# dyollb/segmantic

Measured on AMD Instinct MI355X. Metric: 3D UNet train voxels/s on 128^3 bf16, higher is better.
Workload: dtype bf16

## Files before the change

segmantic_amd/csrc/conv_ring3_impl.h:

```cpp
#pragma once
#include "conv_ring_impl.h"

namespace segmi {

struct Ring3Geom {
  static constexpr int TD = 4, TH = 8, TW = 16, HH = TH + 2, HW = TW + 2;
  static constexpr int ROWB = 32;
  static constexpr int PLANE_ROWS = HH * HW;
  static constexpr int PLANE_B = PLANE_ROWS * ROWB;
  static constexpr int PLANE_CH = PLANE_ROWS * 2;
  static constexpr int GROUP_CH = TD * PLANE_CH;
  static constexpr int GROUP_B = GROUP_CH * 16 + 512;
  static constexpr int NG = 3;
  static constexpr int RING_B = NG * GROUP_B;
  static constexpr int NPIECE = (GROUP_CH + 63) / 64;
  static constexpr int NDMA = (NPIECE + 3) / 4;
  static constexpr int TFS_OFF = RING_B, BPRM_OFF = TFS_OFF + 128, DUMP_OFF = BPRM_OFF + 256;
  static constexpr int LDS_BYTES = DUMP_OFF + 256 * 16;
};

__device__ __forceinline__ void ring3_dma16(const __amdgpu_buffer_rsrc_t rs, unsigned lds_addr, unsigned voff,
                                            unsigned soff) {
  unsigned keep;
  asm volatile(
      "s_mov_b32 %0, m0\n\ts_mov_b32 m0, %1\n\ts_nop 0\n\tbuffer_load_dwordx4 %2, %3, %4 offen lds\n\ts_mov_b32 m0, %0"
      : "=&s"(keep)
      : "s"(lds_addr), "v"(voff), "s"(rs), "s"(soff)
      : "memory");
}

template <typename T, int MODE>
__global__ __launch_bounds__(256, 2) void conv_ring3_kernel(ConvParams p) {
  using G = Ring3Geom;
  constexpr int J = 5;
  constexpr int NIT = 6 * J;
  constexpr unsigned kOob = 0x80000000u;
  extern __shared__ __attribute__((aligned(16))) char smem[];
  const int tid = threadIdx.x, lane = tid & 63;
  const int wave = __builtin_amdgcn_readfirstlane(tid >> 6);
  const int g = lane >> 4, r = lane & 15;

  int t = blockIdx.x;
  if (p.xcd) t = (t & 7) * (gridDim.x >> 3) + (t >> 3);
  const int seg = t % p.tz; t /= p.tz;
  const int txi = t % p.tx; t /= p.tx;
  const int tyi = t % p.ty;
  const int n = t / p.ty;
  const int oy0 = tyi * G::TH, ox0 = txi * G::TW;
  const int nt0 = blockIdx.y;
  const int total_steps = (p.Do + G::TD - 1) / G::TD;
  const int seg_steps = (total_steps + p.tz - 1) / p.tz;
  const int z0 = seg * seg_steps * G::TD;
  const int nsteps_z = total_steps - seg * seg_steps < seg_steps ? total_steps - seg * seg_steps : seg_steps;

  constexpr bool PLAIN = MODE == 0;
  constexpr bool BSUM = MODE == 4;
  constexpr bool has_alpha = (MODE & 1) != 0;
  constexpr bool want_stats = (MODE & 2) != 0;
  const T* resp = (const T*)p.res;
  const bool res_in = resp && p.res == p.in && p.ldr == p.ldi && p.Cin == p.Cout;
  const bool res_ext = resp && !res_in;

  frag_t wreg[3][J];
#pragma unroll
  for (int kd = 0; kd < 3; ++kd)
#pragma unroll
    for (int j = 0; j < J; ++j) {
      wreg[kd][j] = frag_t{0u, 0u, 0u, 0u};
      const int t9 = 2 * j + (g >> 1);
      if (t9 <= 8) {
        const int tap = kd * 9 + t9;
        const int sp = tap >> 1, gp = (tap & 1) * 2 + (g & 1);
        wreg[kd][j] = *reinterpret_cast<const frag_t*>(
            (const char*)p.wfrag + (((int64_t)sp * p.ntiles_total + nt0) * 64 + gp * 16 + r) * 16);
      }
    }
  int lb[J];
#pragma unroll
  for (int j = 0; j < J; ++j) {
    int t9 = 2 * j + (g >> 1);
    if (t9 > 8) t9 = 8;
    lb[j] = ((t9 / 3) * G::HW + t9 % 3 + r) * G::ROWB + (g & 1) * 16 + wave * 2 * G::HW * G::ROWB;
  }

  const int64_t plane_stride = (int64_t)p.Hi * p.Wi * p.ldi * (int64_t)sizeof(T);
  const unsigned plane_b32 = (unsigned)plane_stride;
  const char* img = (const char*)p.in + (int64_t)n * p.Di * plane_stride;
  const __amdgpu_buffer_rsrc_t rs_in =
      __builtin_amdgcn_make_buffer_rsrc((void*)img, 0, (int)((unsigned)p.Di * plane_b32), 0x00020000);
  unsigned goff[G::NDMA];
  unsigned gpl = 0;
  bool xy_inside = true;
#pragma unroll
  for (int mi = 0; mi < G::NDMA; ++mi) {
    const int i = 64 * (wave + 4 * mi) + lane;
    const int pl = i / G::PLANE_CH, rem = i % G::PLANE_CH;
    const int row = rem >> 1, ch = rem & 1;
    const int y = oy0 - 1 + row / G::HW, x = ox0 - 1 + row % G::HW;
    const bool ok = i < G::GROUP_CH && (unsigned)y < (unsigned)p.Hi && (unsigned)x < (unsigned)p.Wi;
    goff[mi] = ok ? (unsigned)pl * plane_b32 + (unsigned)((y * p.Wi + x) * p.ldi * (int)sizeof(T) + ch * 16) : kOob;
    gpl |= (unsigned)((pl & 3) | (ok ? 0 : 8)) << (4 * mi);
    xy_inside = xy_inside && (ok || i >= G::GROUP_CH);
  }
  const bool wave_inside = __builtin_amdgcn_readfirstlane(__all(xy_inside) ? 1 : 0) != 0;
  const unsigned lds0 = (unsigned)(uintptr_t)smem;
  const unsigned lds_wave = (unsigned)(1024 * wave);
  const bool last_piece = wave + 4 * (G::NDMA - 1) < G::NPIECE;
  auto dma_group = [&](unsigned gbase, int zfirst) {
    const unsigned soff = (unsigned)zfirst * plane_b32;
#pragma unroll
    for (int mi = 0; mi < G::NDMA; ++mi)
      if (mi < G::NDMA - 1 || last_piece) ring3_dma16(rs_in, lds0 + gbase + lds_wave + 4096u * mi, goff[mi], soff);
  };

  const bool in_tf = p.in_scale != nullptr;
  const bool in_act = in_tf && p.in_alpha != nullptr;
  float* tfs = reinterpret_cast<float*>(smem + G::TFS_OFF);
  if (in_tf && tid < 32) tfs[tid] = tid < 16 ? p.in_scale[tid] : p.in_shift[tid - 16];
  float in_alpha = in_act ? *p.in_alpha : 0.f;
  touch_s(in_alpha);
  const bool in_act01 = in_act && in_alpha >= 0.f && in_alpha <= 1.f;
  auto transform_group = [&](unsigned gbase, int zrem) {
    const int tfo = (lane & 1) * 32;
    float sc[8], sh[8];
    const char* tb = reinterpret_cast<const char*>(tfs);
#pragma unroll
    for (int e = 0; e < 8; e += 4) {
      *reinterpret_cast<f32x4*>(&sc[e]) = *reinterpret_cast<const f32x4*>(tb + tfo + e * 4);
      *reinterpret_cast<f32x4*>(&sh[e]) = *reinterpret_cast<const f32x4*>(tb + 64 + tfo + e * 4);
    }
    const unsigned mine = gbase + lds_wave + 16u * lane;
    const bool fast = zrem >= G::TD && wave_inside;
    auto run = [&](auto tf, auto dst) {
      frag_t raw[G::NDMA - 1];
#pragma unroll
      for (int mi = 0; mi < G::NDMA - 1; ++mi) raw[mi] = *reinterpret_cast<const frag_t*>(smem + mine + 4096u * mi);
      frag_t rawl = frag_t{0u, 0u, 0u, 0u};
      if (last_piece) rawl = *reinterpret_cast<const frag_t*>(smem + mine + 4096u * (G::NDMA - 1));
#pragma unroll
      for (int mi = 0; mi < G::NDMA - 1; ++mi)
        *reinterpret_cast<frag_t*>(smem + dst(mi, mine + 4096u * mi)) = tf(raw[mi]);
      const unsigned al = last_piece ? dst(G::NDMA - 1, mine + 4096u * (G::NDMA - 1)) : (unsigned)(G::DUMP_OFF + tid * 16);
      *reinterpret_cast<frag_t*>(smem + al) = tf(rawl);
    };
    auto with_dst = [&](auto tf) {
      if (fast) run(tf, [&](int, unsigned a) { return a; });
      else run(tf, [&](int mi, unsigned a) {
        const unsigned nib = (gpl >> (4 * mi)) & 15u;
        const bool keep = nib < 8u && (int)nib < zrem;
        return keep ? a : (unsigned)(G::DUMP_OFF + tid * 16);
      });
    };
    if (in_act01) with_dst([&](frag_t v) { return bn_prelu01_h8<T>(v, sc, sh, in_alpha); });
    else with_dst([&](frag_t v) { return bn_prelu_h8<T>(v, sc, sh, in_alpha, in_act); });
  };

  {
    const unsigned dst0 = 2u * G::GROUP_B + 2u * G::PLANE_B;
#pragma unroll
    for (int mi = 0; mi < 3; ++mi) {
      const int i = 64 * (wave + 4 * mi) + lane;
      const int pl = i / G::PLANE_CH, rem = i % G::PLANE_CH;
      const int row = rem >> 1, ch = rem & 1;
      const int z = z0 - 1 + pl, y = oy0 - 1 + row / G::HW, x = ox0 - 1 + row % G::HW;
      const bool ok = (unsigned)z < (unsigned)p.Di && (unsigned)y < (unsigned)p.Hi && (unsigned)x < (unsigned)p.Wi;
      const unsigned vo = ok ? (unsigned)z * plane_b32 + (unsigned)((y * p.Wi + x) * p.ldi * (int)sizeof(T) + ch * 16) : kOob;
      if (i < 2 * G::PLANE_CH) ring3_dma16(rs_in, lds0 + dst0 + 1024u * (wave + 4 * mi), vo, 0u);
    }
    dma_group(0u, z0 + 1);
    if (in_tf) {
      asm volatile("s_waitcnt vmcnt(0)" ::: "memory");
      __syncthreads();
      const int tfo = (lane & 1) * 32;
      float sc[8], sh[8];
#pragma unroll
      for (int e = 0; e < 8; ++e) { sc[e] = tfs[tfo / 4 + e]; sh[e] = tfs[16 + tfo / 4 + e]; }
#pragma unroll
      for (int mi = 0; mi < 3; ++mi) {
        const int i = 64 * (wave + 4 * mi) + lane;
        const int pl = i / G::PLANE_CH, row = (i % G::PLANE_CH) >> 1;
        const int z = z0 - 1 + pl, y = oy0 - 1 + row / G::HW, x = ox0 - 1 + row % G::HW;
        const bool ok = i < 2 * G::PLANE_CH && (unsigned)z < (unsigned)p.Di && (unsigned)y < (unsigned)p.Hi &&
                        (unsigned)x < (unsigned)p.Wi;
        if (ok) {
          frag_t* q = reinterpret_cast<frag_t*>(smem + dst0 + 16u * i);
          *q = bn_prelu_h8<T>(*q, sc, sh, in_alpha, in_act);
        }
      }
      transform_group(0u, p.Di - (z0 + 1));
    }
    asm volatile("s_waitcnt vmcnt(0) lgkmcnt(0)" ::: "memory");
    __syncthreads();
  }

  f32x4 bias4 = f32x4{0.f, 0.f, 0.f, 0.f};
  if (p.bias) bias4 = *reinterpret_cast<const f32x4*>(p.bias + nt0 * 16 + 4 * g);
  touch_v(bias4);
  float alpha = has_alpha ? *p.alpha : 0.f;
  touch_s(alpha);
  const bool alpha01 = has_alpha && alpha >= 0.f && alpha <= 1.f;
  f32x4 ssum = f32x4{0.f, 0.f, 0.f, 0.f}, ssq = ssum;
  f32x4 bs0 = ssum, bs1 = ssum, bs2 = ssum;
  float* bprm = reinterpret_cast<float*>(smem + G::BPRM_OFF);
  float balpha = 1.f;
  if constexpr (BSUM) {
    if (tid < 64) {
      const int which = tid / 16, ch = nt0 * 16 + tid % 16;
      const float mean = p.bmean[ch], istd = p.binvstd[ch];
      const float sc = istd * (p.bgamma ? p.bgamma[ch] : 1.f);
      bprm[tid] = which == 0 ? mean : which == 1 ? istd : which == 2 ? sc : fmaf(-mean, sc, p.bbeta ? p.bbeta[ch] : 0.f);
    }
    balpha = p.balpha ? *p.balpha : 1.f;
    touch_s(balpha);
    __syncthreads();
  }
  const bool b_has_alpha = BSUM && p.balpha != nullptr;
  const T* bxp = (const T*)p.bx;
  T* outp = (T*)p.out;
  const int co = nt0 * 16 + 4 * g;
  unsigned o_off[2], r_off[2], b_off[2];
  bool row_ok[2];
#pragma unroll
  for (int ro = 0; ro < 2; ++ro) {
    const int oy = oy0 + 2 * wave + ro, ox = ox0 + r;
    row_ok[ro] = oy < p.Ho && ox < p.Wo;
    o_off[ro] = row_ok[ro] ? (unsigned)((oy * p.Wo + ox) * p.ldo + co) * (unsigned)sizeof(T) : kOob;
    r_off[ro] = row_ok[ro] ? (unsigned)((oy * p.Wo + ox) * p.ldr + co) * (unsigned)sizeof(T) : kOob;
    b_off[ro] = row_ok[ro] ? (unsigned)((oy * p.Wo + ox) * p.ldbx + co) * (unsigned)sizeof(T) : kOob;
  }
  const int64_t oplane = (int64_t)p.Ho * p.Wo * p.ldo, rplane = (int64_t)p.Ho * p.Wo * p.ldr;
  const int64_t bplane = (int64_t)p.Ho * p.Wo * p.ldbx;
  const unsigned oplane_b = (unsigned)(oplane * (int64_t)sizeof(T)), rplane_b = (unsigned)(rplane * (int64_t)sizeof(T)),
                 bplane_b = (unsigned)(bplane * (int64_t)sizeof(T));
  const __amdgpu_buffer_rsrc_t rs_out = __builtin_amdgcn_make_buffer_rsrc(
      (void*)(outp + (int64_t)n * p.Do * oplane), 0, (int)((unsigned)p.Do * oplane_b), 0x00020000);
  const __amdgpu_buffer_rsrc_t rs_res = __builtin_amdgcn_make_buffer_rsrc(
      (void*)(res_ext ? resp + (int64_t)n * p.Do * rplane : (const T*)p.out), 0, res_ext ? (int)((unsigned)p.Do * rplane_b) : 0,
      0x00020000);
  const __amdgpu_buffer_rsrc_t rs_bx = __builtin_amdgcn_make_buffer_rsrc(
      (void*)(BSUM ? bxp + (int64_t)n * p.Do * bplane : (const T*)p.out), 0, BSUM ? (int)((unsigned)p.Do * bplane_b) : 0,
      0x00020000);

  unsigned g_prev = 2u * G::GROUP_B, g_cur = 0u, g_next = (unsigned)G::GROUP_B;
  for (int step = 0; step < nsteps_z; ++step) {
    const int zb = step * G::TD;
    const bool more = step + 1 < nsteps_z;
    if (more) dma_group(g_next, z0 + zb + 5);
    typedef typename Raw4<T>::type raw4_t;
    raw4_t resv[4][2];
    if (res_ext) {
#pragma unroll
      for (int zi = 0; zi < 4; ++zi)
#pragma unroll
        for (int ro = 0; ro < 2; ++ro)
          resv[zi][ro] = __builtin_amdgcn_raw_buffer_load_b64(rs_res, r_off[ro], (unsigned)(z0 + zb + zi) * rplane_b, 0);
    }
    raw4_t bxv[BSUM ? 4 : 1][2];
    auto fetch_bx = [&](int zi) {
#pragma unroll
      for (int ro = 0; ro < 2; ++ro)
        bxv[BSUM ? zi : 0][ro] =
            __builtin_amdgcn_raw_buffer_load_b64(rs_bx, b_off[ro], (unsigned)(z0 + zb + zi) * bplane_b, 0);
    };
    if constexpr (BSUM) { fetch_bx(0); fetch_bx(1); fetch_bx(2); fetch_bx(3); }

    int bp[J], bc[J];
#pragma unroll
    for (int j = 0; j < J; ++j) { bp[j] = lb[j] + (int)g_prev; bc[j] = lb[j] + (int)g_cur; }
    f32x4 acc[4][2];
    constexpr int PD = MODE == 4 ? 3 : 4;
    frag_t a[PD + 1][2];
    auto issue = [&](int it, frag_t (&dst)[2]) {
      const int c = it / J, j = it % J;
      const char* base = smem + (c < 2 ? bp[j] + (c + 2) * G::PLANE_B : bc[j] + (c - 2) * G::PLANE_B);
      dst[0] = *reinterpret_cast<const frag_t*>(base);
      dst[1] = *reinterpret_cast<const frag_t*>(base + G::HW * G::ROWB);
    };
#pragma unroll
    for (int q = 0; q < PD; ++q) issue(q, a[q]);
#pragma unroll
    for (int it = 0; it < NIT; ++it) {
      if (it + PD < NIT) issue(it + PD, a[(it + PD) % (PD + 1)]);
      __builtin_amdgcn_sched_barrier(0);
      const int c = it / J, j = it % J;
#pragma unroll
      for (int kd = 0; kd < 3; ++kd) {
        const int zi = c - kd;
        if (zi >= 0 && zi < 4) {
          const bool first = kd == 0 && j == 0;
          const f32x4 zero = f32x4{0.f, 0.f, 0.f, 0.f};
          acc[zi][0] = mma16<T>(wreg[kd][j], a[it % (PD + 1)][0], first ? zero : acc[zi][0]);
          acc[zi][1] = mma16<T>(wreg[kd][j], a[it % (PD + 1)][1], first ? zero : acc[zi][1]);
        }
      }
      __builtin_amdgcn_sched_barrier(0);
    }
    if (in_tf && more) {
      asm volatile("s_waitcnt vmcnt(0)" ::: "memory");
      transform_group(g_next, p.Di - (z0 + zb + 5));
    }
    if (res_in) {
#pragma unroll
      for (int zi = 0; zi < 4; ++zi)
#pragma unroll
        for (int ro = 0; ro < 2; ++ro) {
          const int c = zi + 1;
          const unsigned pb = c < 2 ? g_prev + (c + 2) * G::PLANE_B : g_cur + (c - 2) * G::PLANE_B;
          resv[zi][ro] = *reinterpret_cast<const raw4_t*>(
              smem + pb + ((2 * wave + ro + 1) * G::HW + r + 1) * G::ROWB + (4 * g) * (int)sizeof(T));
        }
    }
    if (resp) {
#pragma unroll
      for (int zi = 0; zi < 4; ++zi)
#pragma unroll
        for (int ro = 0; ro < 2; ++ro) touch_v(resv[zi][ro]);
    }
    f32x4 bsc4, bsh4, bmean4;
    if constexpr (BSUM) {
#pragma unroll
      for (int zi = 0; zi < 4; ++zi)
#pragma unroll
        for (int ro = 0; ro < 2; ++ro) touch_v(bxv[zi][ro]);
      bsc4 = *reinterpret_cast<const f32x4*>(bprm + 2 * 16 + 4 * g);
      bsh4 = *reinterpret_cast<const f32x4*>(bprm + 3 * 16 + 4 * g);
      bmean4 = *reinterpret_cast<const f32x4*>(bprm + 4 * g);
    }
#pragma unroll
    for (int zi = 0; zi < 4; ++zi) {
      const int oz = z0 + zb + zi;
      const unsigned opoff = (unsigned)oz * oplane_b;
      const bool zin_out = oz < p.Do;
#pragma unroll
      for (int ro = 0; ro < 2; ++ro) {
        f32x4 v = acc[zi][ro] + bias4;
        const bool valid = zin_out & row_ok[ro];
        if (want_stats) {
          const f32x4 vm = valid ? v : f32x4{0.f, 0.f, 0.f, 0.f};
          ssum += vm;
          ssq += vm * vm;
        }
        if (has_alpha) {
          if (alpha01) {
#pragma unroll
            for (int e = 0; e < 4; ++e) v[e] = fmaxf(v[e], alpha * v[e]);
          } else {
#pragma unroll
            for (int e = 0; e < 4; ++e) v[e] = v[e] > 0.f ? v[e] : alpha * v[e];
          }
        }
        if (resp) v += Raw4<T>::cvt(resv[zi][ro]);
        u32x2 o;
        o[0] = H16<T>::pack2(v[0], v[1]);
        o[1] = H16<T>::pack2(v[2], v[3]);
        __builtin_amdgcn_raw_buffer_store_b64(o, rs_out, o_off[ro], opoff, 0);
        if constexpr (BSUM) {
          f32x4 d = Raw4<T>::cvt(o);
          if (!valid) d = f32x4{0.f, 0.f, 0.f, 0.f};
          const f32x4 xr = Raw4<T>::cvt(bxv[zi][ro]);
#pragma unroll
          for (int e = 0; e < 4; ++e) {
            const float z = fmaf(xr[e], bsc4[e], bsh4[e]);
            float dz = d[e];
            if (b_has_alpha && !(z > 0.f)) { bs2[e] = fmaf(d[e], z, bs2[e]); dz = balpha * d[e]; }
            bs0[e] += dz;
            bs1[e] = fmaf(dz, xr[e] - bmean4[e], bs1[e]);
          }
        }
      }
    }
    const unsigned gp = g_prev;
    g_prev = g_cur; g_cur = g_next; g_next = gp;
    asm volatile("s_waitcnt vmcnt(8) lgkmcnt(0)" ::: "memory");
    __builtin_amdgcn_s_barrier();
  }

  if constexpr (BSUM) {
    float* red = reinterpret_cast<float*>(smem);
#pragma unroll
    for (int e = 0; e < 4; ++e) {
      const float a0 = row16_sum(bs0[e]);
      const float a1 = row16_sum(bs1[e]);
      const float a2 = row16_sum(bs2[e]);
      if (r == 0) {
        red[(wave * 3 + 0) * 16 + 4 * g + e] = a0;
        red[(wave * 3 + 1) * 16 + 4 * g + e] = a1;
        red[(wave * 3 + 2) * 16 + 4 * g + e] = a2;
      }
    }
    __syncthreads();
    if (tid < 48) {
      const int which = tid / 16, ch = tid % 16;
      float sacc = 0.f;
#pragma unroll
      for (int w = 0; w < 4; ++w) sacc += red[(w * 3 + which) * 16 + ch];
      if (which == 1) sacc *= bprm[16 + ch];
      fin_store(&p.bpart[((int64_t)blockIdx.x * 3 + which) * p.Cout + nt0 * 16 + ch], sacc);
    }
    fin_tail_run<BnBwdFin, 256, offsetof(ConvParams, ft), offsetof(ConvParams, bbfin)>(p.bpart, smem);
  }
  if (want_stats) {
    float* red = reinterpret_cast<float*>(smem);
#pragma unroll
    for (int e = 0; e < 4; ++e) {
      const float a0 = row16_sum(ssum[e]);
      const float b0 = row16_sum(ssq[e]);
      if (r == 0) {
        red[(wave * 2 + 0) * 16 + 4 * g + e] = a0;
        red[(wave * 2 + 1) * 16 + 4 * g + e] = b0;
      }
    }
    __syncthreads();
    if (tid < 32) {
      const int which = tid / 16, ch = tid % 16;
      float sacc = 0.f;
#pragma unroll
      for (int w = 0; w < 4; ++w) sacc += red[(w * 2 + which) * 16 + ch];
      fin_store(&p.stats[((int64_t)blockIdx.x * 2 + which) * p.Cout + nt0 * 16 + ch], sacc);
    }
    fin_tail_run<BnFin, 256, offsetof(ConvParams, ft), offsetof(ConvParams, bfin)>(p.stats, smem);
  }
}

static inline bool conv_ring3_ok(const ConvParams& p) {
  return conv_ring3_shape_ok(p.Cin, p.Cout, p.in, p.out, p.Di, p.Hi, p.Wi, p.ldi, p.Do, p.Ho, p.Wo, p.ldo, p.ldr, p.ldbx);
}

template <typename T, int MODE>
static int launch_conv_ring3_k(ConvParams p, hipStream_t st) {
  using G = Ring3Geom;
  p.tz = conv_ring_zsplit(DtypeOf<T>::value, p.Cin, 3, 1, p.N, p.Do, p.Ho, p.Wo);
  p.ty = cdiv(p.Ho, G::TH);
  p.tx = cdiv(p.Wo, G::TW);
  dim3 grid((unsigned)(p.N * p.ty * p.tx * p.tz), (unsigned)(p.Cout / 16));
  p.xcd = grid.x <= 512 && grid.x % 8 == 0;
  constexpr bool kStats = (MODE & 2) != 0, kBsum = MODE == 4;
  p.fin_on = p.fin_on && (kStats || kBsum);
  (void)fin_tail_arm(p, grid, 256, (kBsum ? 3 : 2) * p.Cout, G::LDS_BYTES);
  auto kern = conv_ring3_kernel<T, MODE>;
  static bool attr_done = false;
  if (!attr_done) {
    (void)hipFuncSetAttribute(reinterpret_cast<const void*>(kern), hipFuncAttributeMaxDynamicSharedMemorySize,
                              G::LDS_BYTES);
    attr_done = true;
  }
  hipLaunchKernelGGL(kern, grid, 256, G::LDS_BYTES, st, p);
  SEGMI_LAUNCH_CHECK("conv3d_fwd(ring3)");
  return SEGMI_OK;
}

template <typename T>
static int launch_conv_ring3(const ConvParams& p, hipStream_t st) {
  if (p.bpart && !p.alpha && !p.stats && p.Cout == 16) return launch_conv_ring3_k<T, 4>(p, st);
  switch ((p.alpha ? 1 : 0) | (p.stats ? 2 : 0)) {
    case 0: return launch_conv_ring3_k<T, 0>(p, st);
    case 1: return launch_conv_ring3_k<T, 1>(p, st);
    case 2: return launch_conv_ring3_k<T, 2>(p, st);
    default: return launch_conv_ring3_k<T, 3>(p, st);
  }
}

}
```

segmantic_amd/csrc/wgrad_ws_impl.h:

```cpp
#pragma once
#include <type_traits>
#include "wgrad_impl.h"

namespace segmi {

__device__ __forceinline__ void ws_barrier() {
  asm volatile("s_waitcnt lgkmcnt(0)\n\ts_barrier" ::: "memory");
}

template <typename T, int KS, int S, int CTO, int CTI, int TD, int TH, int TW>
__global__ __launch_bounds__(768) void wgrad_ws_kernel(WgradParams p) {
  using G = WgradGeom<T, KS, S, CTO, CTI, TD, TH, TW>;
  constexpr int BUF = (G::LDS_BYTES + 255) / 256 * 256;
  extern __shared__ __attribute__((aligned(16))) char smem[];
  const int tid = threadIdx.x;
  const int wave = __builtin_amdgcn_readfirstlane(tid >> 6);

  const int cochunk = blockIdx.y / p.ci_chunks, cichunk = blockIdx.y % p.ci_chunks;
  const int co0 = cochunk * 16 * CTO, ci0 = cichunk * 16 * CTI;

  const int nx = gridDim.x, bid = blockIdx.x;
  const int cols = p.ty * p.tx;
  const int nunits = p.N * p.zs * cols;
  int u_begin, u_end, u_stride;
  if ((nx & 7) == 0) {
    const int xcd = bid & 7, slot = bid >> 3;
    u_begin = (int)((int64_t)nunits * xcd / 8) + slot;
    u_end = (int)((int64_t)nunits * (xcd + 1) / 8);
    u_stride = nx >> 3;
  } else {
    u_begin = bid; u_end = nunits; u_stride = nx;
  }
  auto unit_len = [&](int u) {
    const int seg = (u / cols) % p.zs;
    const int left = p.tz - seg * p.zper;
    return left < p.zper ? left : p.zper;
  };
  int niter = 0;
  for (int u = u_begin; u < u_end; u += u_stride) niter += unit_len(u);

  constexpr bool ROWS = KS == 3 && S == 1 && CTO == 1 && CTI == 1 && TW == 16 && TH == 8;
  if constexpr (ROWS) {
    if (wave < 4) {
      typedef unsigned u32x8 __attribute__((ext_vector_type(8)));
      const int lane = tid & 63;
      const int g = lane >> 4, i16 = lane & 15;
      const int q = i16 >> 2, pp = i16 & 3;
      const int lane_line = (4 * g + q) * 32 + 8 * pp;
      const int ybase = lane_line + (2 * wave * TW) * G::YROWB;
      const int xbase = G::YBYTES + lane_line + (2 * wave * G::HW) * G::XROWB;
      f32x4 acc[27];
#pragma unroll
      for (int t = 0; t < 27; ++t) acc[t] = f32x4{0.f, 0.f, 0.f, 0.f};
      constexpr int NSTRIP = G::HD * 3;
      constexpr int PD = 2;
      auto read_strip = [&](const char* buf, int sidx) {
        const int c = sidx / 3, dx = sidx % 3;
        u32x8 st;
#pragma unroll
        for (int j = 0; j < 4; ++j) {
          const s16x4 r = __builtin_amdgcn_ds_read_tr16_b64_v4i16(
              (lds_s16x4*)(buf + xbase + ((c * G::HH + j) * G::HW + dx) * G::XROWB));
          const u32x2 r2 = __builtin_bit_cast(u32x2, r);
          st[2 * j] = r2[0]; st[2 * j + 1] = r2[1];
        }
        return st;
      };
      ws_barrier();
      for (int it = 0; it < niter; ++it) {
        const char* buf = smem + (it & 1) * BUF;
        frag_t af[TD];
#pragma unroll
        for (int z = 0; z < TD; ++z) {
          const s16x4 lo = __builtin_amdgcn_ds_read_tr16_b64_v4i16(
              (lds_s16x4*)(buf + ybase + ((z * TH) * TW) * G::YROWB));
          const s16x4 hi = __builtin_amdgcn_ds_read_tr16_b64_v4i16(
              (lds_s16x4*)(buf + ybase + ((z * TH + 1) * TW) * G::YROWB));
          const u32x2 l2 = __builtin_bit_cast(u32x2, lo), h2 = __builtin_bit_cast(u32x2, hi);
          af[z] = frag_t{l2[0], l2[1], h2[0], h2[1]};
        }
        u32x8 strip[PD + 1];
#pragma unroll
        for (int s0 = 0; s0 < PD; ++s0) strip[s0] = read_strip(buf, s0);
#pragma unroll
        for (int sidx = 0; sidx < NSTRIP; ++sidx) {
          if (sidx + PD < NSTRIP) strip[(sidx + PD) % (PD + 1)] = read_strip(buf, sidx + PD);
          __builtin_amdgcn_sched_barrier(0);
          const int c = sidx / 3, dx = sidx % 3;
          const u32x8 st = strip[sidx % (PD + 1)];
          const frag_t bfs[3] = {__builtin_shufflevector(st, st, 0, 1, 2, 3),
                                 __builtin_shufflevector(st, st, 2, 3, 4, 5),
                                 __builtin_shufflevector(st, st, 4, 5, 6, 7)};
#pragma unroll
          for (int kh = 0; kh < 3; ++kh) {
            const frag_t bf = bfs[kh];
#pragma unroll
            for (int kd = 0; kd < 3; ++kd) {
              const int z = c - kd;
              if (z >= 0 && z < TD) {
                const int t = (kd * 3 + kh) * 3 + dx;
                acc[t] = mma16<T>(af[z], bf, acc[t]);
              }
            }
          }
          __builtin_amdgcn_sched_barrier(0);
        }
        ws_barrier();
      }
      f32x4* red = reinterpret_cast<f32x4*>(smem);
      if (wave >= 2) {
#pragma unroll
        for (int t = 0; t < 27; ++t) red[((wave - 2) * 27 + t) * 64 + lane] = acc[t];
      }
      ws_barrier();
      if (wave < 2) {
#pragma unroll
        for (int t = 0; t < 27; ++t) acc[t] += red[(wave * 27 + t) * 64 + lane];
      }
      ws_barrier();
      if (wave == 1) {
#pragma unroll
        for (int t = 0; t < 27; ++t) red[t * 64 + lane] = acc[t];
      }
      ws_barrier();
      if (wave == 0) {
        float* slab = p.partials + (int64_t)blockIdx.x * p.Cout * p.Cin * 27;
#pragma unroll
        for (int t = 0; t < 27; ++t) {
          const f32x4 v = acc[t] + red[t * 64 + lane];
#pragma unroll
          for (int e = 0; e < 4; ++e) {
            const int co = co0 + 4 * g + e, ci = ci0 + i16;
            slab[((int64_t)co * p.Cin + ci) * 27 + t] = v[e];
          }
        }
      }
      return;
    }
  }
  if (!ROWS && wave < 4) {
    const int lane = tid & 63;
    const int g = lane >> 4, i16 = lane & 15;
    f32x4 acc[G::NTW][CTO][CTI];
#pragma unroll
    for (int a = 0; a < G::NTW; ++a)
#pragma unroll
      for (int b = 0; b < CTO; ++b)
#pragma unroll
        for (int c = 0; c < CTI; ++c) acc[a][b][c] = f32x4{0.f, 0.f, 0.f, 0.f};
    int tapoff[G::NTW];
#pragma unroll
    for (int ti = 0; ti < G::NTW; ++ti) {
      int tap = wave + 4 * ti;
      if (tap > G::NTAPS - 1) tap = G::NTAPS - 1;
      const int kd = tap / (KS * KS), kh = (tap / KS) % KS, kw = tap % KS;
      tapoff[ti] = ((kd * G::HH + kh) * G::HW + kw) * G::XROWB;
    }
    const int q = i16 >> 2, pp = i16 & 3;
    const int v = 4 * g + q;
    const int ylane = v * G::YROWB + 8 * pp;
    const int xlane = ((v / TW) * S * G::HW + (v % TW) * S) * G::XROWB + 8 * pp;

    frag_t af[2][CTO], bf[2][G::NTW][CTI];
    auto read_group = [&](const char* ysm, const char* xsm, int lg, frag_t (&a)[CTO], frag_t (&b)[G::NTW][CTI]) {
#pragma unroll
      for (int ct = 0; ct < CTO; ++ct) {
        const s16x4 lo = __builtin_amdgcn_ds_read_tr16_b64_v4i16(
            (lds_s16x4*)(ysm + ylane + (2 * lg) * 16 * G::YROWB + ct * 32));
        const s16x4 hi = __builtin_amdgcn_ds_read_tr16_b64_v4i16(
            (lds_s16x4*)(ysm + ylane + (2 * lg + 1) * 16 * G::YROWB + ct * 32));
        const u32x2 l2 = __builtin_bit_cast(u32x2, lo), h2 = __builtin_bit_cast(u32x2, hi);
        a[ct] = frag_t{l2[0], l2[1], h2[0], h2[1]};
      }
      const int r0 = wg_line_row<S, TH, TW, G::HH, G::HW>(2 * lg) * G::XROWB;
      const int r1 = wg_line_row<S, TH, TW, G::HH, G::HW>(2 * lg + 1) * G::XROWB;
#pragma unroll
      for (int ti = 0; ti < G::NTW; ++ti)
#pragma unroll
        for (int c = 0; c < CTI; ++c) {
          const s16x4 lo = __builtin_amdgcn_ds_read_tr16_b64_v4i16(
              (lds_s16x4*)(xsm + xlane + tapoff[ti] + r0 + c * 32));
          const s16x4 hi = __builtin_amdgcn_ds_read_tr16_b64_v4i16(
              (lds_s16x4*)(xsm + xlane + tapoff[ti] + r1 + c * 32));
          const u32x2 l2 = __builtin_bit_cast(u32x2, lo), h2 = __builtin_bit_cast(u32x2, hi);
          b[ti][c] = frag_t{l2[0], l2[1], h2[0], h2[1]};
        }
    };
    constexpr int NKG = G::NL / 2;
    static_assert(NKG % 2 == 0, "k-groups come in pairs (register-set parity)");
    ws_barrier();
    for (int it = 0; it < niter; ++it) {
      char* ysm = smem + (it & 1) * BUF;
      char* xsm = ysm + G::YBYTES;
      read_group(ysm, xsm, 0, af[0], bf[0]);
#pragma unroll
      for (int lg = 0; lg < NKG; ++lg) {
        if (lg + 1 < NKG) read_group(ysm, xsm, lg + 1, af[(lg + 1) & 1], bf[(lg + 1) & 1]);
        __builtin_amdgcn_sched_barrier(0);
#pragma unroll
        for (int ti = 0; ti < G::NTW; ++ti)
#pragma unroll
          for (int ct = 0; ct < CTO; ++ct)
#pragma unroll
            for (int c = 0; c < CTI; ++c)
              acc[ti][ct][c] = mma16<T>(af[lg & 1][ct], bf[lg & 1][ti][c], acc[ti][ct][c]);
        __builtin_amdgcn_sched_barrier(0);
      }
      ws_barrier();
    }
    float* slab = p.partials + (int64_t)blockIdx.x * p.Cout * p.Cin * G::NTAPS;
#pragma unroll
    for (int ti = 0; ti < G::NTW; ++ti) {
      const int tap = wave + 4 * ti;
      if (tap < G::NTAPS) {
#pragma unroll
        for (int ct = 0; ct < CTO; ++ct)
#pragma unroll
          for (int c = 0; c < CTI; ++c)
#pragma unroll
            for (int e = 0; e < 4; ++e) {
              const int co = co0 + ct * 16 + 4 * g + e, ci = ci0 + c * 16 + i16;
              slab[((int64_t)co * p.Cin + ci) * G::NTAPS + tap] = acc[ti][ct][c][e];
            }
      }
    }
    return;
  }

  constexpr int PT = 512;
  const int ptid = tid - 256;
  constexpr int NLY = (G::NV * G::YCPR + PT - 1) / PT, NLX = (G::XROWS * G::XCPR + PT - 1) / PT;
  static_assert(NLX <= 32, "one validity bit per staged X chunk");
  static_assert(G::HD < 127 && G::HH < 127 && G::HW < 127 && TD < 127 && TH < 127 && TW < 127, "packed coordinates");
  unsigned y_goff[NLY], x_goff[NLX], y_pk[NLY], x_pk[NLX];
  constexpr int OV = S == 1 ? G::HD - TD * S : 0;
  constexpr int OV_SRC = TD * S * G::HH * G::HW * G::XROWB;
  static_assert(OV >= 0 && OV < G::HD, "overlap planes");
  unsigned x_ov = 0u;
#pragma unroll
  for (int k = 0; k < NLY; ++k) {
    const int i = ptid + PT * k;
    const int v = i / G::YCPR, ch = i % G::YCPR;
    const int vz = v / (TW * TH), vy = (v / TW) % TH, vx = v % TW;
    const bool has = i < G::NV * G::YCPR;
    y_goff[k] = has ? (unsigned)(((vz * p.Hy + vy) * p.Wy + vx) * p.ldy * (int)sizeof(T) + ch * 16) : 0u;
    y_pk[k] = has ? (unsigned)(vz | (vy << 8) | (vx << 16)) : 0x7f7f7fu;
  }
  const unsigned x_center = (unsigned)(((G::PAD * p.Hx + G::PAD) * p.Wx + G::PAD) * p.ldx * (int)sizeof(T));
#pragma unroll
  for (int k = 0; k < NLX; ++k) {
    const int i = ptid + PT * k;
    const int v = i / G::XCPR, ch = i % G::XCPR;
    const int hx = v % G::HW, hy = (v / G::HW) % G::HH, hz = v / (G::HW * G::HH);
    const bool has = i < G::XROWS * G::XCPR;
    x_goff[k] = has ? (unsigned)(((hz * p.Hx + hy) * p.Wx + hx) * p.ldx * (int)sizeof(T) + ch * 16) : x_center;
    x_pk[k] = has ? (unsigned)(hz | (hy << 8) | (hx << 16)) : 0x7f7f7fu;
    x_ov |= (has && hz < OV) ? (1u << k) : 0u;
  }
  const bool in_tf = p.in_scale != nullptr;
  const bool in_act = in_tf && p.in_alpha != nullptr;
  float tsc[8], tsh[8];
  float in_alpha = in_act ? *p.in_alpha : 0.f;
#pragma unroll
  for (int e = 0; e < 8; ++e) {
    const int ch = ci0 + (ptid % G::XCPR) * 8 + e;
    tsc[e] = in_tf ? p.in_scale[ch] : 1.f;
    tsh[e] = in_tf ? p.in_shift[ch] : 0.f;
  }
  static_assert(PT % G::XCPR == 0, "a thread's X chunks share their channel offset");
  const int mode = !in_tf ? 0 : (in_act ? (in_alpha >= 0.f && in_alpha <= 1.f ? 3 : 2) : 1);
  const __amdgpu_buffer_rsrc_t xrs = __builtin_amdgcn_make_buffer_rsrc((void*)p.x, 0, p.x_bytes, 0x00020000);
  const __amdgpu_buffer_rsrc_t yrs = __builtin_amdgcn_make_buffer_rsrc((void*)p.dy, 0, p.y_bytes, 0x00020000);
  constexpr unsigned OOB = 0xfffffff0u;

  int cur_u = u_begin, cur_z = 0, cur_zend = 0, cur_t = 0, cur_zbeg = 0;
  unsigned ybase = 0u, xbase = 0u;
  bool xy_border = false;
  unsigned ylim_xy = 0u, xlo_xy = 0u, xhi_xy = 0u;
  const unsigned ystep = (unsigned)((int64_t)TD * p.Hy * p.Wy * p.ldy * 2);
  const unsigned xstep = (unsigned)((int64_t)TD * S * p.Hx * p.Wx * p.ldx * 2);
  auto clamp7 = [](int v) { return (unsigned)(v < 0 ? 0 : (v > 126 ? 126 : v)); };
  auto open_unit = [&](int u) {
    int t = u;
    const int ux = t % p.tx; t /= p.tx;
    const int uy = t % p.ty; t /= p.ty;
    const int seg = t % p.zs;
    const int n = t / p.zs;
    cur_z = seg * p.zper;
    cur_zbeg = cur_z;
    cur_zend = cur_z + unit_len(u);
    const int oz0 = cur_z * TD, oy0 = uy * TH, ox0 = ux * TW;
    const int iz0 = oz0 * S - G::PAD, iy0 = oy0 * S - G::PAD, ix0 = ox0 * S - G::PAD;
    ybase = (unsigned)((((((int64_t)n * p.Dy + oz0) * p.Hy + oy0) * p.Wy + ox0) * p.ldy + co0) * 2);
    xbase = (unsigned)((((((int64_t)n * p.Dx + iz0) * p.Hx + iy0) * p.Wx + ix0) * p.ldx + ci0) * 2);
    xy_border = iy0 < 0 || ix0 < 0 || iy0 + G::HH > p.Hx || ix0 + G::HW > p.Wx || oy0 + TH > p.Hy || ox0 + TW > p.Wy;
    ylim_xy = (clamp7(p.Hy - oy0 - 1) << 8) | (clamp7(p.Wy - ox0 - 1) << 16);
    xlo_xy = (clamp7(-iy0) << 8) | (clamp7(-ix0) << 16);
    xhi_xy = (clamp7(p.Hx - iy0 - 1) << 8) | (clamp7(p.Wx - ix0 - 1) << 16);
  };
  auto advance = [&]() {
    ++cur_t;
    if (cur_t < niter) {
      if (++cur_z == cur_zend) { cur_u += u_stride; open_unit(cur_u); }
      else { ybase += ystep; xbase += xstep; }
    }
  };
  if (niter > 0) open_unit(cur_u);

  auto fetch = [&](frag_t (&ry)[NLY], frag_t (&rx)[NLX], unsigned& xmask, bool& cont) {
    const int oz0 = cur_z * TD, iz0 = oz0 * S - G::PAD;
    const bool border = xy_border || iz0 < 0 || iz0 + G::HD > p.Dx || oz0 + TD > p.Dy;
    cont = OV > 0 && cur_z != cur_zbeg;
    const unsigned skip = cont ? x_ov : 0u;
    if (!border) {
#pragma unroll
      for (int k = 0; k < NLY; ++k) ry[k] = __builtin_amdgcn_raw_buffer_load_b128(yrs, y_goff[k], ybase, 0);
      if (!cont) {
#pragma unroll
        for (int k = 0; k < NLX; ++k) rx[k] = __builtin_amdgcn_raw_buffer_load_b128(xrs, x_goff[k], xbase, 0);
      } else {
#pragma unroll
        for (int k = 0; k < NLX; ++k) {
          if ((PT * (k + 1) - 1) / G::XCPR < OV * G::HH * G::HW) continue;
          rx[k] = __builtin_amdgcn_raw_buffer_load_b128(xrs, ((skip >> k) & 1u) ? OOB : xbase + x_goff[k], 0, 0);
        }
      }
    } else {
      const unsigned ylim = clamp7(p.Dy - oz0 - 1) | ylim_xy;
      const unsigned xlo = clamp7(-iz0) | xlo_xy;
      const unsigned xhi = clamp7(p.Dx - iz0 - 1) | xhi_xy;
#pragma unroll
      for (int k = 0; k < NLY; ++k) {
        const bool ok = (((ylim | 0x808080u) - y_pk[k]) & 0x808080u) == 0x808080u;
        ry[k] = __builtin_amdgcn_raw_buffer_load_b128(yrs, ok ? ybase + y_goff[k] : OOB, 0, 0);
      }
      unsigned xm = 0u;
#pragma unroll
      for (int k = 0; k < NLX; ++k) {
        const unsigned t1 = (x_pk[k] | 0x808080u) - xlo, t2 = (xhi | 0x808080u) - x_pk[k];
        const bool ok = (t1 & t2 & 0x808080u) == 0x808080u;
        rx[k] = __builtin_amdgcn_raw_buffer_load_b128(xrs, ok && !((skip >> k) & 1u) ? xbase + x_goff[k] : OOB, 0, 0);
        xm |= ok ? (1u << k) : 0u;
      }
      xmask = xm;
    }
    advance();
    return border;
  };
  auto commit_with = [&](int buf, const frag_t (&ry)[NLY], const frag_t (&rx)[NLX], unsigned xmask, bool cont, auto tf,
                         auto masked) {
    char* const ysm = smem + buf * BUF;
    char* const xsm = ysm + G::YBYTES;
    const char* const xprev = smem + (buf ^ 1) * BUF + G::YBYTES + OV_SRC;
    const unsigned skip = cont ? x_ov : 0u;
#pragma unroll
    for (int k = 0; k < NLY; ++k) {
      const int i = ptid + PT * k;
      if (i < G::NV * G::YCPR)
        *reinterpret_cast<frag_t*>(ysm + (i / G::YCPR) * G::YROWB + (i % G::YCPR) * 16) = ry[k];
    }
#pragma unroll
    for (int k = 0; k < NLX; ++k) {
      const int i = ptid + PT * k;
      if (i < G::XROWS * G::XCPR) {
        const int lo = (i / G::XCPR) * G::XROWB + (i % G::XCPR) * 16;
        frag_t val = rx[k];
        if ((skip >> k) & 1u) {
          val = *reinterpret_cast<const frag_t*>(xprev + lo);
        } else if constexpr (decltype(masked)::value) {
          if ((xmask >> k) & 1u) val = tf(val);
        } else {
          val = tf(val);
        }
        *reinterpret_cast<frag_t*>(xsm + lo) = val;
      }
    }
  };
  auto commit = [&](int buf, const frag_t (&ry)[NLY], const frag_t (&rx)[NLX], unsigned xmask, bool border, bool cont) {
    using Yes = std::integral_constant<bool, true>;
    using No = std::integral_constant<bool, false>;
    if (mode == 0) { commit_with(buf, ry, rx, xmask, cont, [](frag_t v) { return v; }, No{}); return; }
    auto with_mask = [&](auto tf) {
      if (border) commit_with(buf, ry, rx, xmask, cont, tf, Yes{});
      else commit_with(buf, ry, rx, xmask, cont, tf, No{});
    };
    if (mode == 3) with_mask([&](frag_t v) { return bn_prelu01_h8<T>(v, tsc, tsh, in_alpha); });
    else if (mode == 2) with_mask([&](frag_t v) { return bn_prelu_h8<T>(v, tsc, tsh, in_alpha, true); });
    else with_mask([&](frag_t v) { return bn_prelu_h8<T>(v, tsc, tsh, 0.f, false); });
  };

  frag_t ryA[NLY], rxA[NLX], ryB[NLY], rxB[NLX];
  unsigned xmA = 0u, xmB = 0u;
  bool bdA = false, bdB = false;
  bool ctA = false, ctB = false, ctC = false;
  if (niter > 0) {
    bdA = fetch(ryA, rxA, xmA, ctA);
    if (niter > 1) bdB = fetch(ryB, rxB, xmB, ctB);
    commit(0, ryA, rxA, xmA, bdA, ctA);
    if (niter > 2) bdA = fetch(ryA, rxA, xmA, ctC);
    ctA = ctC;
  }
  ws_barrier();
  for (int it = 0; it < niter; it += 2) {
    if (it + 1 < niter) commit(1, ryB, rxB, xmB, bdB, ctB);
    if (it + 3 < niter) bdB = fetch(ryB, rxB, xmB, ctB);
    ws_barrier();
    if (it + 1 >= niter) break;
    if (it + 2 < niter) commit(0, ryA, rxA, xmA, bdA, ctA);
    if (it + 4 < niter) bdA = fetch(ryA, rxA, xmA, ctA);
    ws_barrier();
  }
  if constexpr (ROWS) { ws_barrier(); ws_barrier(); ws_barrier(); }
}

template <int KS, int S, int CTO, int CTI, int TD, int TH, int TW>
static constexpr int wgrad_ws_lds() {
  using G = WgradGeom<bf16_t, KS, S, CTO, CTI, TD, TH, TW>;
  return 2 * ((G::LDS_BYTES + 255) / 256 * 256);
}

template <typename T, int KS, int S, int CTO, int CTI, int TD, int TH, int TW>
static int launch_wgrad_ws_cfg(WgradParams p, int gx, hipStream_t st) {
  using G = WgradGeom<T, KS, S, CTO, CTI, TD, TH, TW>;
  constexpr int LDS = wgrad_ws_lds<KS, S, CTO, CTI, TD, TH, TW>();
  static_assert(LDS <= 160 * 1024, "two tile buffers must fit the CU's LDS");
  p.tz = cdiv(p.Dy, TD);
  p.ty = cdiv(p.Hy, TH);
  p.tx = cdiv(p.Wy, TW);
  p.ntiles = p.N * p.tz * p.ty * p.tx;
  int zs = 1;
  while (p.N * p.ty * p.tx * zs < gx && 2 * (zs + 1) <= p.tz) ++zs;
  p.zper = cdiv(p.tz, zs);
  p.zs = cdiv(p.tz, p.zper);
  SEGMI_CHECK_ARG((int64_t)G::HD * p.Hx * p.Wx * p.ldx * 2 < (1ll << 31) &&
                      (int64_t)TD * p.Hy * p.Wy * p.ldy * 2 < (1ll << 31),
                  "conv3d_wgrad: plane too large for the MFMA kernel's 32-bit tile offsets");
  const int64_t xb = (((int64_t)p.N * p.Dx * p.Hx * p.Wx - 1) * p.ldx + p.Cin) * 2;
  const int64_t yb = (((int64_t)p.N * p.Dy * p.Hy * p.Wy - 1) * p.ldy + p.Cout) * 2;
  SEGMI_CHECK_ARG(xb < 0xfff00000ll && yb < 0xfff00000ll, "conv3d_wgrad(ws): tensor beyond the 4 GB buffer range");
  p.x_bytes = (unsigned)xb; p.y_bytes = (unsigned)yb;
  p.ci_chunks = p.Cin / (16 * CTI);
  const int co_chunks = p.Cout / (16 * CTO);
  dim3 grid((unsigned)gx, (unsigned)(co_chunks * p.ci_chunks));
  auto kern = wgrad_ws_kernel<T, KS, S, CTO, CTI, TD, TH, TW>;
  static bool attr_done = false;
  if (!attr_done) {
    (void)hipFuncSetAttribute(reinterpret_cast<const void*>(kern),
                              hipFuncAttributeMaxDynamicSharedMemorySize, LDS);
    attr_done = true;
  }
  hipLaunchKernelGGL(kern, grid, 768, LDS, st, p);
  SEGMI_LAUNCH_CHECK("conv3d_wgrad(ws)");
  return SEGMI_OK;
}

}
```

Before: 3.642 billion.

## Stage wgrad dY tiles via direct buffer-to-LDS DMA instead of registers

The warp-specialized wgrad producer waves now load the dY tile straight into LDS with buffer_load ... lds, instead of loading it into VGPRs and writing it out with ds_write. This frees the ryA/ryB register arrays and removes the LDS store traffic for dY. Explicit vmcnt waits sized to the number of outstanding X loads are added before each barrier so the DMA lands in time. The shared DMA helper is moved into a common header. The main risk is ordering: the vmcnt accounting has to be exact, and the extra waits could serialize the prefetch.

New measurement: 3.647 billion (median of 2 runs). No clear change (+0.1%).

```diff
diff --git a/segmantic_amd/csrc/conv_ring3_impl.h b/segmantic_amd/csrc/conv_ring3_impl.h
--- a/segmantic_amd/csrc/conv_ring3_impl.h
+++ b/segmantic_amd/csrc/conv_ring3_impl.h
@@ -1,5 +1,6 @@
 #pragma once
 #include "conv_ring_impl.h"
+#include "lds_dma.h"
 
 namespace segmi {
 
@@ -19,16 +20,6 @@
   static constexpr int LDS_BYTES = DUMP_OFF + 256 * 16;
 };
 
-__device__ __forceinline__ void ring3_dma16(const __amdgpu_buffer_rsrc_t rs, unsigned lds_addr, unsigned voff,
-                                            unsigned soff) {
-  unsigned keep;
-  asm volatile(
-      "s_mov_b32 %0, m0\n\ts_mov_b32 m0, %1\n\ts_nop 0\n\tbuffer_load_dwordx4 %2, %3, %4 offen lds\n\ts_mov_b32 m0, %0"
-      : "=&s"(keep)
-      : "s"(lds_addr), "v"(voff), "s"(rs), "s"(soff)
-      : "memory");
-}
-
 template <typename T, int MODE>
 __global__ __launch_bounds__(256, 2) void conv_ring3_kernel(ConvParams p) {
   using G = Ring3Geom;
@@ -110,7 +101,7 @@
     const unsigned soff = (unsigned)zfirst * plane_b32;
 #pragma unroll
     for (int mi = 0; mi < G::NDMA; ++mi)
-      if (mi < G::NDMA - 1 || last_piece) ring3_dma16(rs_in, lds0 + gbase + lds_wave + 4096u * mi, goff[mi], soff);
+      if (mi < G::NDMA - 1 || last_piece) lds_dma16(rs_in, lds0 + gbase + lds_wave + 4096u * mi, goff[mi], soff);
   };
 
   const bool in_tf = p.in_scale != nullptr;
@@ -165,7 +156,7 @@
       const int z = z0 - 1 + pl, y = oy0 - 1 + row / G::HW, x = ox0 - 1 + row % G::HW;
       const bool ok = (unsigned)z < (unsigned)p.Di && (unsigned)y < (unsigned)p.Hi && (unsigned)x < (unsigned)p.Wi;
       const unsigned vo = ok ? (unsigned)z * plane_b32 + (unsigned)((y * p.Wi + x) * p.ldi * (int)sizeof(T) + ch * 16) : kOob;
-      if (i < 2 * G::PLANE_CH) ring3_dma16(rs_in, lds0 + dst0 + 1024u * (wave + 4 * mi), vo, 0u);
+      if (i < 2 * G::PLANE_CH) lds_dma16(rs_in, lds0 + dst0 + 1024u * (wave + 4 * mi), vo, 0u);
     }
     dma_group(0u, z0 + 1);
     if (in_tf) {
diff --git a/segmantic_amd/csrc/lds_dma.h b/segmantic_amd/csrc/lds_dma.h
--- /dev/null
+++ b/segmantic_amd/csrc/lds_dma.h
@@ -0,0 +1,22 @@
+#pragma once
+#include "common.h"
+
+namespace segmi {
+
+__device__ __forceinline__ void lds_dma16(const __amdgpu_buffer_rsrc_t rs, unsigned lds_addr, unsigned voff,
+                                          unsigned soff) {
+  unsigned keep;
+  asm volatile(
+      "s_mov_b32 %0, m0\n\ts_mov_b32 m0, %1\n\ts_nop 0\n\tbuffer_load_dwordx4 %2, %3, %4 offen lds\n\ts_mov_b32 m0, %0"
+      : "=&s"(keep)
+      : "s"(lds_addr), "v"(voff), "s"(rs), "s"(soff)
+      : "memory");
+}
+
+template <int N>
+__device__ __forceinline__ void vm_wait() {
+  static_assert(N >= 0 && N < 64, "vmcnt is a 6-bit counter");
+  asm volatile("s_waitcnt vmcnt(%0)" ::"n"(N) : "memory");
+}
+
+}
diff --git a/segmantic_amd/csrc/wgrad_ws_impl.h b/segmantic_amd/csrc/wgrad_ws_impl.h
--- a/segmantic_amd/csrc/wgrad_ws_impl.h
+++ b/segmantic_amd/csrc/wgrad_ws_impl.h
@@ -1,5 +1,6 @@
 #pragma once
 #include <type_traits>
+#include "lds_dma.h"
 #include "wgrad_impl.h"
 
 namespace segmi {
@@ -233,6 +234,10 @@
   static_assert(NLX <= 32, "one validity bit per staged X chunk");
   static_assert(G::HD < 127 && G::HH < 127 && G::HW < 127 && TD < 127 && TH < 127 && TW < 127, "packed coordinates");
   unsigned y_goff[NLY], x_goff[NLX], y_pk[NLY], x_pk[NLX];
+  constexpr int YCH = G::NV * G::YCPR;
+  static_assert(G::YROWB == 16 * G::YCPR && YCH % 64 == 0, "dY pieces: lane-linear, whole waves");
+  const int pw = wave - 4;
+  const unsigned lds0 = (unsigned)(uintptr_t)smem;
   constexpr int OV = S == 1 ? G::HD - TD * S : 0;
   constexpr int OV_SRC = TD * S * G::HH * G::HW * G::XROWB;
   static_assert(OV >= 0 && OV < G::HD, "overlap planes");
@@ -307,14 +312,19 @@
   };
   if (niter > 0) open_unit(cur_u);
 
-  auto fetch = [&](frag_t (&ry)[NLY], frag_t (&rx)[NLX], unsigned& xmask, bool& cont) {
+  constexpr int NSKIP = [] {
+    int n = 0;
+    for (int k = 0; k < NLX; ++k) n += (PT * (k + 1) - 1) / G::XCPR < OV * G::HH * G::HW ? 1 : 0;
+    return n;
+  }();
+  auto fetch = [&](frag_t (&rx)[NLX], unsigned& xmask, bool& cont, unsigned& yb, unsigned& yl, int& nld) {
     const int oz0 = cur_z * TD, iz0 = oz0 * S - G::PAD;
     const bool border = xy_border || iz0 < 0 || iz0 + G::HD > p.Dx || oz0 + TD > p.Dy;
     cont = OV > 0 && cur_z != cur_zbeg;
     const unsigned skip = cont ? x_ov : 0u;
+    yb = ybase;
+    nld = NLX;
     if (!border) {
-#pragma unroll
-      for (int k = 0; k < NLY; ++k) ry[k] = __builtin_amdgcn_raw_buffer_load_b128(yrs, y_goff[k], ybase, 0);
       if (!cont) {
 #pragma unroll
         for (int k = 0; k < NLX; ++k) rx[k] = __builtin_amdgcn_raw_buffer_load_b128(xrs, x_goff[k], xbase, 0);
@@ -324,16 +334,12 @@
           if ((PT * (k + 1) - 1) / G::XCPR < OV * G::HH * G::HW) continue;
           rx[k] = __builtin_amdgcn_raw_buffer_load_b128(xrs, ((skip >> k) & 1u) ? OOB : xbase + x_goff[k], 0, 0);
         }
+        nld = NLX - NSKIP;
       }
     } else {
-      const unsigned ylim = clamp7(p.Dy - oz0 - 1) | ylim_xy;
+      yl = clamp7(p.Dy - oz0 - 1) | ylim_xy;
       const unsigned xlo = clamp7(-iz0) | xlo_xy;
       const unsigned xhi = clamp7(p.Dx - iz0 - 1) | xhi_xy;
-#pragma unroll
-      for (int k = 0; k < NLY; ++k) {
-        const bool ok = (((ylim | 0x808080u) - y_pk[k]) & 0x808080u) == 0x808080u;
-        ry[k] = __builtin_amdgcn_raw_buffer_load_b128(yrs, ok ? ybase + y_goff[k] : OOB, 0, 0);
-      }
       unsigned xm = 0u;
 #pragma unroll
       for (int k = 0; k < NLX; ++k) {
@@ -347,18 +353,29 @@
     advance();
     return border;
   };
-  auto commit_with = [&](int buf, const frag_t (&ry)[NLY], const frag_t (&rx)[NLX], unsigned xmask, bool cont, auto tf,
-                         auto masked) {
-    char* const ysm = smem + buf * BUF;
-    char* const xsm = ysm + G::YBYTES;
+  auto dma_y = [&](int buf, unsigned yb, bool border, unsigned yl) {
+    yb = __builtin_amdgcn_readfirstlane(yb);
+#pragma unroll
+    for (int k = 0; k < NLY; ++k) {
+      if (64 * pw + PT * k >= YCH) continue;
+      const unsigned dst = lds0 + (unsigned)(buf * BUF + 16 * (64 * pw + PT * k));
+      if (!border) {
+        lds_dma16(yrs, dst, y_goff[k], yb);
+      } else {
+        const bool ok = (((yl | 0x808080u) - y_pk[k]) & 0x808080u) == 0x808080u;
+        lds_dma16(yrs, dst, ok ? yb + y_goff[k] : OOB, 0u);
+      }
+    }
+  };
+  auto dma_wait = [&](int nld) {
+    if (nld == NLX) vm_wait<NLX>();
+    else if (NSKIP > 0 && nld == NLX - NSKIP) vm_wait<NLX - NSKIP>();
+    else vm_wait<0>();
+  };
+  auto commit_with = [&](int buf, const frag_t (&rx)[NLX], unsigned xmask, bool cont, auto tf, auto masked) {
+    char* const xsm = smem + buf * BUF + G::YBYTES;
     const char* const xprev = smem + (buf ^ 1) * BUF + G::YBYTES + OV_SRC;
     const unsigned skip = cont ? x_ov : 0u;
-#pragma unroll
-    for (int k = 0; k < NLY; ++k) {
-      const int i = ptid + PT * k;
-      if (i < G::NV * G::YCPR)
-        *reinterpret_cast<frag_t*>(ysm + (i / G::YCPR) * G::YROWB + (i % G::YCPR) * 16) = ry[k];
-    }
 #pragma unroll
     for (int k = 0; k < NLX; ++k) {
       const int i = ptid + PT * k;
@@ -376,38 +393,47 @@
       }
     }
   };
-  auto commit = [&](int buf, const frag_t (&ry)[NLY], const frag_t (&rx)[NLX], unsigned xmask, bool border, bool cont) {
+  auto commit = [&](int buf, const frag_t (&rx)[NLX], unsigned xmask, bool border, bool cont) {
     using Yes = std::integral_constant<bool, true>;
     using No = std::integral_constant<bool, false>;
-    if (mode == 0) { commit_with(buf, ry, rx, xmask, cont, [](frag_t v) { return v; }, No{}); return; }
+    if (mode == 0) { commit_with(buf, rx, xmask, cont, [](frag_t v) { return v; }, No{}); return; }
     auto with_mask = [&](auto tf) {
-      if (border) commit_with(buf, ry, rx, xmask, cont, tf, Yes{});
-      else commit_with(buf, ry, rx, xmask, cont, tf, No{});
+      if (border) commit_with(buf, rx, xmask, cont, tf, Yes{});
+      else commit_with(buf, rx, xmask, cont, tf, No{});
     };
     if (mode == 3) with_mask([&](frag_t v) { return bn_prelu01_h8<T>(v, tsc, tsh, in_alpha); });
     else if (mode == 2) with_mask([&](frag_t v) { return bn_prelu_h8<T>(v, tsc, tsh, in_alpha, true); });
     else with_mask([&](frag_t v) { return bn_prelu_h8<T>(v, tsc, tsh, 0.f, false); });
   };
 
-  frag_t ryA[NLY], rxA[NLX], ryB[NLY], rxB[NLX];
+  frag_t rxA[NLX], rxB[NLX];
   unsigned xmA = 0u, xmB = 0u;
+  unsigned ybA = 0u, ybB = 0u, ylA = 0u, ylB = 0u;
   bool bdA = false, bdB = false;
   bool ctA = false, ctB = false, ctC = false;
+  int nld = 0;
   if (niter > 0) {
-    bdA = fetch(ryA, rxA, xmA, ctA);
-    if (niter > 1) bdB = fetch(ryB, rxB, xmB, ctB);
-    commit(0, ryA, rxA, xmA, bdA, ctA);
-    if (niter > 2) bdA = fetch(ryA, rxA, xmA, ctC);
+    bdA = fetch(rxA, xmA, ctA, ybA, ylA, nld);
+    if (niter > 1) bdB = fetch(rxB, xmB, ctB, ybB, ylB, nld);
+    dma_y(0, ybA, bdA, ylA);
+    commit(0, rxA, xmA, bdA, ctA);
+    nld = 0;
+    if (niter > 2) bdA = fetch(rxA, xmA, ctC, ybA, ylA, nld);
     ctA = ctC;
   }
+  dma_wait(nld);
   ws_barrier();
   for (int it = 0; it < niter; it += 2) {
-    if (it + 1 < niter) commit(1, ryB, rxB, xmB, bdB, ctB);
-    if (it + 3 < niter) bdB = fetch(ryB, rxB, xmB, ctB);
+    nld = 0;
+    if (it + 1 < niter) { dma_y(1, ybB, bdB, ylB); commit(1, rxB, xmB, bdB, ctB); }
+    if (it + 3 < niter) bdB = fetch(rxB, xmB, ctB, ybB, ylB, nld);
+    dma_wait(nld);
     ws_barrier();
     if (it + 1 >= niter) break;
-    if (it + 2 < niter) commit(0, ryA, rxA, xmA, bdA, ctA);
-    if (it + 4 < niter) bdA = fetch(ryA, rxA, xmA, ctA);
+    nld = 0;
+    if (it + 2 < niter) { dma_y(0, ybA, bdA, ylA); commit(0, rxA, xmA, bdA, ctA); }
+    if (it + 4 < niter) bdA = fetch(rxA, xmA, ctA, ybA, ylA, nld);
+    dma_wait(nld);
     ws_barrier();
   }
   if constexpr (ROWS) { ws_barrier(); ws_barrier(); ws_barrier(); }
```
